# Starfish-develop/Starfish

Measured on AMD Instinct MI355X. Metric: log-likelihood evals/sec, 4096-pixel order, batch=128 walkers, higher is better.
Workload: dtype f64; 1 GPU; cfg2: synthetic single order N_pix=4096, 8 eigenspectra, M=27, N_f=8192, 1 global + 1 local kernel, all 13 parameters thawed, batch=128 walkers per GPU; global_batch=128, units_per_gpu=128, parallelism=(order x walker) units sharded x1, one process per GPU, no data-path collective

## Files before the change

include/starfish_amd.h:

```cpp
#ifndef STARFISH_AMD_H
#define STARFISH_AMD_H

#include <stddef.h>
#include <stdint.h>

#ifdef __cplusplus
extern "C" {
#endif

#define SF_OK 0
#define SF_EINVAL (-1)
#define SF_ENOMEM (-2)
#define SF_EHIP (-3)
#define SF_ENODEV (-4)

#define SF_INFO_OUT_OF_GRID (-1)
#define SF_INFO_BAD_VSINI (-2)
#define SF_INFO_BAD_WEIGHT_COV (-3)
#define SF_INFO_BANDWIDTH (-4)
#define SF_INFO_INTERNAL (-5)

#define SF_INFO_NAN (-6)

#define SF_JITTER 1e-10
// ... 144 lines not shown
int sf_banded_max_halfwidth(const sf_ctx* ctx);
int sf_banded_window_halfwidth(const sf_ctx* ctx);
size_t sf_banded_workspace_bytes(const sf_ctx* ctx, const sf_model_desc* model, int B, int halfwidth);
int sf_loglike_banded_batch(sf_ctx* ctx, const sf_model_desc* model, int B, const double* d_params,
                            int halfwidth, double* d_lnl, double* d_logdet, double* d_sqmah,
                            double* d_resid, double* d_log_scale, int* d_info, void* d_work,
                            size_t work_bytes, void* stream);

int sf_band_logdet_gram_batch(const double* d_band, int n, int halfwidth, int ldb, int64_t stride,
                              int batch, const double* d_rhs, int nrhs, int ldr, int64_t rhs_stride,
                              double* d_logdet, double* d_gram, int* d_info, void* stream);

int sf_profile_enable(int on);
int sf_profile_read(double* ms_by_stage, double* gemm_flops, long* gemm_launches, long* calls);

int sf_emulator_v11_build(const double* d_grid, int M, int P, int m, const double* d_hyper, const double* d_iphiphi,
                          double* d_A, int npad, int lda, void* stream);

int sf_emulator_v11_build_batch(const double* d_grid, int M, int P, int m, const double* d_hyper, int hyper_stride, int B,
                                const double* d_iphiphi, double* d_A, int npad, int lda, int64_t stride, int lower_only,
                                const double* d_w_hat, double* d_R, int ldr, void* stream);

size_t sf_emulator_loglike_workspace_bytes(int M, int m, int B);
int sf_emulator_loglike_batch(const double* d_grid, int M, int P, int m, const double* d_hyper, int hyper_stride, int B,
                              const double* d_iphiphi, const double* d_w_hat, double* d_lnl, double* d_logdet,
                              double* d_sqmah, int* d_info, void* d_work, size_t work_bytes, void* stream);

int sf_persistent_potrf(int enable);

int sf_persistent_potrf_status(long long* h_out8);

int sf_debug_cholesky_sequence(int mode);

int sf_debug_clock_probe(long long* d_out2, long long wall_ticks_100mhz, void* stream);

int sf_debug_stream_write(double* d_dst, size_t count, double value, void* stream);

#ifdef __cplusplus
}
#endif
#endif
```

starfish_amd/_lib.py:

```python

import ctypes as C
import os

_HERE = os.path.dirname(os.path.abspath(__file__))
LIB_PATH = os.path.join(_HERE, "libstarfish_amd.so")
if os.environ.get("SF_LIB_PATH"):
    import warnings

    LIB_PATH = os.environ["SF_LIB_PATH"]
    warnings.warn(f"starfish_amd: SF_LIB_PATH overrides the packaged library: loading {LIB_PATH}", RuntimeWarning)

c_double_p = C.POINTER(C.c_double)
c_int_p = C.POINTER(C.c_int)


class OrderDesc(C.Structure):
    _fields_ = [
        ("n", C.c_int32),
        ("nf", C.c_int32),
        ("m", C.c_int32),
        ("n_grid", C.c_int32),
        ("M", C.c_int32),
        ("reserved", C.c_int32),
        ("wave", c_double_p),
# ... 118 lines not shown
    ),
    "sf_emulator_joint_batch": (
        C.c_int,
        [_VP, C.POINTER(ModelDesc), C.c_int, _VP, _VP, _VP, _VP, _VP, C.c_size_t, _VP],
    ),
    "sf_loglike_batch": (
        C.c_int,
        [_VP, C.POINTER(ModelDesc), C.c_int, _VP, _VP, _VP, _VP, _VP, _VP, _VP, _VP, C.c_size_t, _VP],
    ),
    "sf_multi_workspace_bytes": (C.c_size_t, [C.POINTER(Segment), C.c_int, C.POINTER(ModelDesc)]),
    "sf_loglike_multi_batch": (
        C.c_int,
        [C.POINTER(Segment), C.c_int, C.POINTER(ModelDesc), _VP, _VP, _VP, _VP, _VP, _VP, C.c_size_t, _VP],
    ),
    "sf_multi_workspace_bytes_md": (C.c_size_t, [C.POINTER(Segment), C.c_int, C.POINTER(C.POINTER(ModelDesc))]),
    "sf_loglike_multi_batch_md": (
        C.c_int,
        [C.POINTER(Segment), C.c_int, C.POINTER(C.POINTER(ModelDesc)), _VP, _VP, _VP, _VP, _VP, _VP, C.c_size_t, _VP],
    ),
    "sf_banded_max_halfwidth": (C.c_int, [_VP]),
    "sf_banded_window_halfwidth": (C.c_int, [_VP]),
    "sf_banded_workspace_bytes": (C.c_size_t, [_VP, C.POINTER(ModelDesc), C.c_int, C.c_int]),
    "sf_loglike_banded_batch": (
        C.c_int,
        [_VP, C.POINTER(ModelDesc), C.c_int, _VP, C.c_int, _VP, _VP, _VP, _VP, _VP, _VP, _VP, C.c_size_t, _VP],
    ),
    "sf_band_logdet_gram_batch": (
        C.c_int,
        [_VP, C.c_int, C.c_int, C.c_int, C.c_int64, C.c_int, _VP, C.c_int, C.c_int, C.c_int64, _VP, _VP, _VP, _VP],
    ),
    "sf_debug_clock_probe": (C.c_int, [_VP, C.c_longlong, _VP]),
    "sf_debug_stream_write": (C.c_int, [_VP, C.c_size_t, C.c_double, _VP]),
    "sf_debug_cholesky_sequence": (C.c_int, [C.c_int]),
    "sf_persistent_potrf": (C.c_int, [C.c_int]),
    "sf_persistent_potrf_status": (C.c_int, [C.POINTER(C.c_longlong)]),
    "sf_profile_enable": (C.c_int, [C.c_int]),
    "sf_profile_read": (C.c_int, [c_double_p, c_double_p, C.POINTER(C.c_long), C.POINTER(C.c_long)]),
}

_lib = None


class StarfishAMDError(RuntimeError):
    """The HIP library is missing, no MI355X is visible, or a C-ABI call failed."""


def load():
    global _lib
    if _lib is not None:
        return _lib
    if not os.path.exists(LIB_PATH):
        raise StarfishAMDError(
            f"{LIB_PATH} not found: build it with `python -c 'import __graft_entry__ as g; g.build()'` "
            "or `make -C starfish_amd/csrc`.  There is no CPU fallback."
        )
    import torch

    lib = C.CDLL(LIB_PATH)
    for name, (res, args) in SIGNATURES.items():
        if not hasattr(lib, name):
            if os.environ.get("SF_LIB_PATH") and os.environ.get("SF_ALLOW_OLD_LIB") == "1":
                import warnings

                warnings.warn(f"starfish_amd: {LIB_PATH} lacks {name} (SF_ALLOW_OLD_LIB=1: skipped)", RuntimeWarning)
                continue
            raise StarfishAMDError(f"{LIB_PATH} does not export {name}: stale or mismatched build of the library "
# ... 27 lines not shown
```

starfish_amd/csrc/sf_chol.hip:

```cpp
#include <atomic>
#include <cstdlib>
#include <type_traits>
#include <vector>

#include "sf_common.h"
#include <stdio.h>
#include "sf_device.h"
#include "sf_chol_tile.h"
#include "sf_chol_host.h"
#include "sf_chol_unfused.h"
#include "sf_chol_diag.h"
#include "sf_chol_sync.h"
#include "sf_chol_solve.h"
#include "sf_chol_apply.h"
#include "sf_chol_panel.h"
#include "sf_chol_wide.h"
#include "sf_chol_seq.h"
#include "sf_chol_band.h"
#include "sf_chol_dataflow.h"

static std::atomic<int> g_chol_sequence{-1};
int sf_set_cholesky_sequence(int mode) {
    if (mode < -1 || mode > 4) {
        sf_set_error("cholesky sequence: -1 automatic, 0 fused panel kernel, 1 unfused, 2 wide (panel pairs), 3 wide then narrow (test aid), 4 dataflow");
        return SF_EINVAL;
    }
    g_chol_sequence.store(mode);
    return SF_OK;
}

#define SF_UNFUSED_BELOW 16
static bool sf_potrf_dataflow_auto(int n, int batch) {
    const int nt = (n + GT - 1) / GT;
    return sf_potrf_dataflow_fits(n, batch) && (long long)batch * nt <= 2048 && batch <= 128 && nt <= 65;
}
static int sf_potrf_pick(int n, int batch) {
    const int sel = g_chol_sequence.load();
    if (sel == 4 && !sf_potrf_dataflow_fits(n, batch)) return 0;
    if (sel >= 0) return sel;
    if (sf_potrf_dataflow_auto(n, batch)) return 4;
    if (n >= 2048 && (long long)batch * ((n + GT - 1) / GT) >= 3400) return 2;
// ... 27 lines not shown
```

starfish_amd/csrc/sf_chol_band.h:

```cpp
#pragma once
#include "sf_chol_host.h"
#include "sf_chol_panel.h"
#include "sf_chol_seq.h"

__global__ __launch_bounds__(256) void k_band_border_rows(const double* __restrict__ rhs0, int64_t srhs0, const double* __restrict__ rhs,
                                                          int64_t srhs, int ldr, int nrhs, int n, int nband, double* __restrict__ A,
                                                          int64_t sA, int lda) {
    const int b = blockIdx.z, r = blockIdx.y, col = blockIdx.x * 256 + threadIdx.x;
    if (col >= nband + 64) return;
    double v = 0.0;
    if (r < nrhs && col < n) v = r == 0 ? rhs0[(int64_t)b * srhs0 + col] : rhs[(int64_t)b * srhs + (int64_t)(r - 1) * ldr + col];
    A[(int64_t)b * sA + (int64_t)(nband + r) * lda + col] = v;
}
__global__ __launch_bounds__(256) void k_band_tiles_finish(const double* __restrict__ A, int64_t sA, int lda, int nband, int nrhs,
                                                           double* __restrict__ logdet, double* __restrict__ gram) {
    __shared__ double red[256];
    const int b = blockIdx.x, tid = threadIdx.x;
    const double* Ab = A + (int64_t)b * sA;
    double acc = 0.0;
    for (int i = tid; i < nband; i += 256) acc += log(Ab[(int64_t)i * lda + i]);
    red[tid] = acc;
    __syncthreads();
    for (int st = 128; st > 0; st >>= 1) {
        if (tid < st) red[tid] += red[tid + st];
// ... 31 lines not shown
    SF_LAUNCH_CHECK();

    const sf_potrf_scratch ws = sf_potrf_scratch_of(work, next, batch);
    auto launch_panel = [&](int k0, int pw, int row0, int nslab, bool border) -> int {
        sf_panel_args g = {};
        g.C = A;
        g.sC = sA;
        g.lda = lda;
        g.n = next;
        g.k0 = k0;
        g.pw = pw;
        g.row0 = row0;
        g.nslab = nslab + (border ? 1 : 0);
        g.slab_step = 1;
        g.Wt = ws.W;
        g.sW = ws.sW;
        g.kband = halfwidth > 0 ? halfwidth : 1;
        g.nband = nband;
        g.xrow0 = border ? nband : 0;
        if (nslab > 0) sf_park(g, ws);
        const long long nblk = (long long)g.nslab * batch;
        if (nblk <= 0) return SF_OK;
        void* tok;
        sf_prof_gemm_begin(s, 2.0 * (double)min(k0, halfwidth + GT) * GT * pw * (double)nblk, &tok);
        hipLaunchKernelGGL((k_chol_panel<false, 0>), dim3((unsigned)nblk), dim3(512), 0, s, g);
        sf_prof_gemm_end(tok);
        SF_LAUNCH_CHECK();
        return SF_OK;
    };
    SF_TRY(launch_panel(0, 0, 0, 1, false));
    for (int k = 0; k < nt; ++k) {
        const int k0 = k * GT;
        const int pw = (nband - k0 < GT) ? nband - k0 : GT;
        SF_TRY(sf_diag_step(ws, A, lda, sA, nullptr, 0, info, nband, k, ws.W, 0, s));
        const int last = (k + wt < nt - 1) ? k + wt : nt - 1;
        SF_TRY(launch_panel(k0, pw, (k + 1) * GT, last - k, true));
    }
    hipLaunchKernelGGL(k_band_tiles_finish, dim3(batch), dim3(256), 0, s, A, sA, lda, nband, nrhs, logdet, gram);
    SF_LAUNCH_CHECK();
    return SF_OK;
}
```

starfish_amd/csrc/sf_chol_dataflow.h:

```cpp
#pragma once
#include "sf_chol_host.h"
#include "sf_chol_diag.h"
#include "sf_chol_sync.h"
#include "sf_chol_panel.h"

struct sf_df_stage {
    int off;
    int St;
    int Sr;
    int thr_pt;
    int thr_rp;
    int dep;
    int fw;
};
struct sf_df_stage_packed {
    int off;
    unsigned short thr_pt, thr_rp, fw;
    unsigned char split;
    signed char dep;
};
static_assert(sizeof(sf_df_stage_packed) == 12, "sf_df_stage_packed");
template <class S>
__host__ __device__ __forceinline__ sf_df_stage sf_df_stage_of(S& x) {
    sf_df_stage r;
// ... 254 lines not shown
        }
        bl = __builtin_amdgcn_readfirstlane(bl);
        i = __builtin_amdgcn_readfirstlane(i);
        sp = __builtin_amdgcn_readfirstlane(sp);
        k = __builtin_amdgcn_readfirstlane(k);
        S = __builtin_amdgcn_readfirstlane(S);
        d = __builtin_amdgcn_readfirstlane(d);
        type = __builtin_amdgcn_readfirstlane(type);
        const int b = bchain >= 0 ? bchain : qcur + SF_DF_QUEUES * bl;
#ifdef SF_TUNING
        if ((a.miss_claims & 2) && type == T_C && b == 0 && k == 2) {
            if (tid == 0)
                while (sf_df_load(a.abort_flag) == 0) __builtin_amdgcn_s_sleep(64);
            __syncthreads();
            continue;
        }
#endif
        const int vb = bchain >= 0 ? (((a.batch - (b & (SF_DF_QUEUES - 1)) + SF_DF_QUEUES - 1) / SF_DF_QUEUES) == a.bq[0] ? 0 : 1) : v;
#ifdef SF_TUNING
        const long long dbg_t0 = wall_clock64();
        long long dbg_t1 = dbg_t0, dbg_top = 0;
#define SF_DF_MARK() dbg_t1 = wall_clock64()
#else
#define SF_DF_MARK()
#endif

        const auto& g = a.p;
        sf_panel_task q = {};
        q.nslab = 1;
        q.slab_step = 1;
        q.abort_flag = a.abort_flag;
        q.lds_int = s_ints + 1;
        q.sW = a.sT;
        auto Wof = [&](int kk) { return a.T + (size_t)(1 + kk) * GT * SF_LDT; };
        auto fpart = [&](int kk, int dd, int SS) {
            return a.part + 2 * region + (((int64_t)((kk & 1) * F + dd - 1) * a.batch + b) * a.pt_cap - (int64_t)b * SS) * (GT * GT);
        };
        int* fcnt = a.fp_cnt + 2 * SF_DF_FRONT_MAX * b;
        bool ok = true;
        int mode = 3, bid = b;
        if (type == T_C || type == T_FR) {
            const int kp = type == T_C ? k - 1 : k;
            const int slab = kp + d;
            if (type == T_C) {
                __builtin_amdgcn_s_setprio(2);
                q.Sout = a.T;
            }
            if (kp < 0) {
                if (tid == 0) __builtin_amdgcn_fence(__ATOMIC_ACQUIRE, "agent");
                __syncthreads();
            } else {
                const sf_df_stage stp = sf_df_stage_of(a.st[vb][kp > 0 ? kp - 1 : 0]);
                const int St = kp >= 1 ? stp.St : 0;
                q.k0 = kp * GT;
                q.pw = min(GT, n - q.k0);
                q.row0 = slab * GT;
                q.Wt = Wof(kp);
                q.ksplit = St;
                q.ktail = St > 0 ? (kp - 1) * (GT / GK) : 0;
                q.part = fpart(kp, d, St);
                bool dready = false;
                ok = sf_df_wait(kp >= 1 ? a.row_L + (size_t)b * nt + slab : nullptr, kp, a.done_top + b, kp,
                                St > 0 ? fcnt + SF_DF_FRONT_MAX * (kp & 1) + d - 1 : nullptr, stp.thr_pt - a.thr_base[vb][kp & 1][d - 1], a.done_D + b, kp + 1, &dready, a.abort_flag,
                                tid, s_ints + 1);
                if (!dready) {
                    q.wflag = a.done_D + b;
                    q.wval = kp + 1;
// ... 498 lines not shown
```

starfish_amd/csrc/sf_chol_host.h:

```cpp
#pragma once
#include "sf_chol_tile.h"

#define SF_TSKEW 40
#define SF_CHIP_WGS 512
#define SF_SPLIT_MAX 8
static size_t sf_split_region_tiles(void) { return 2 * SF_CHIP_WGS; }
__device__ __forceinline__ size_t sf_split_region_tiles_dev(void) { return 2 * SF_CHIP_WGS; }
static int sf_split_policy(long long wgs, int nk) {
    int S = 1;
    while (2 * S <= SF_SPLIT_MAX && wgs * 2 * S <= 384 && nk / (2 * S) >= 8) S *= 2;
    return S;
}
struct sf_potrf_scratch {
    double* T;
    int64_t sT;
    double* W;
    int64_t sW;
    double* part;
    int batch;
    size_t doubles;
    double* Wbuf(int i) const { return W + (size_t)i * batch * sW; }
    size_t Wdoubles() const { return 2 * (size_t)batch * sW; }
    double* Wslot(int k) const { return Wbuf((k >> 1) & 1) + (size_t)(k & 1) * GT * SF_LDT; }
};
static sf_potrf_scratch sf_potrf_scratch_of(double* work, int n, int batch) {
    sf_potrf_scratch w = {};
    const size_t b = (size_t)batch;
    w.sT = (int64_t)(n + SF_NB) * SF_LDT + SF_TSKEW;
    w.sW = (int64_t)SF_NB * SF_LDT + SF_TSKEW;
    w.batch = batch;
    const size_t oT = b * SF_LTB_DOUBLES, oW = oT + b * w.sT, opart = oW + w.Wdoubles() + 64;
    w.doubles = opart + (size_t)(SF_EXEC_GROUPS + 1) * sf_split_region_tiles() * (GT * GT);
    if (work) {
        w.T = work + oT;
        w.W = work + oW;
        w.part = work + opart;
    }
    return w;
}
size_t sf_potrf_work_doubles(int n, int batch) { return sf_potrf_scratch_of(nullptr, n, batch).doubles; }

template <class Args>
static void sf_set_gen(Args& g, const sf_gen_args* gen, int fp) {
    if (!gen) return;
    g.genY = gen->Y - fp;
    g.sY = (int64_t)gen->mpad * gen->ldy;
    g.ldy = gen->ldy;
    g.mpad = gen->mpad;
    g.tilemap = gen->tilemap;
    g.nt128 = gen->nt128;
}
template <class Args>
static Args sf_panel_frame(double* A, int n, int lda, int64_t stride, double* rhs, int ldr, const sf_gen_args* gen, int fp) {
    Args g = {};
    g.C = A;
    g.sC = stride;
// ... 31 lines not shown
```

starfish_amd/csrc/sf_chol_seq.h:

```cpp
#pragma once
#include "sf_chol_host.h"
#include "sf_chol_diag.h"
#include "sf_chol_panel.h"
#include "sf_chol_wide.h"

static int sf_check_front_pad(int fp, int n) {
    if (fp != 0 && (fp != 64 || n % GT != 64)) {
        sf_set_error("potrf: front pad %d does not fit n = %d", fp, n);
        return SF_EINVAL;
    }
    return SF_OK;
}

template <class Args>
static void sf_park(Args& g, const sf_potrf_scratch& ws) {
    g.Sout = ws.T;
    g.sS = ws.sT;
    g.ldS = SF_LDT;
}
static double sf_slab_rows(int n, int row0, int nslab, int step) {
    double rows = 0.0;
    for (int i = 0; i < nslab; ++i) {
        const int r0 = row0 + i * step * GT;
        rows += (n - r0 < GT) ? n - r0 : GT;
    }
    return rows;
}
static int sf_check_grid(long long nblk) {
    if (nblk > 0x7fffffffLL) {
        sf_set_error("panel grid too large");
        return SF_EINVAL;
    }
    return SF_OK;
}

static int sf_panel_split(int k0, int pw, int fp, long long nblk) {
    return pw > 0 ? sf_split_policy(nblk, (k0 > fp ? k0 - fp : 0) / GK) : 1;
}
static int sf_panel_step(sf_panel_args g, const sf_potrf_scratch& ws, int k0, int pw, int row0, int nslab, int step, const double* Wt,
                         bool to_scratch, hipStream_t st, int region, int phase) {
    const int n = g.n, fp = g.fp, batch = ws.batch;
    g.k0 = k0;
    g.pw = pw;
    g.row0 = row0;
    g.nslab = nslab;
    g.slab_step = step;
    g.Wt = Wt;
    g.sW = ws.sW;
    if (to_scratch) {
        sf_park(g, ws);
        g.prio = 1;
    }
    const long long nblk = (long long)nslab * batch;
    SF_TRY(sf_check_grid(nblk));
    const double rows = sf_slab_rows(n, row0, nslab, step);
    const double flops_main = 2.0 * (k0 > fp ? k0 - fp : 0) * rows * pw * batch;
    const double flops_epi = (rows * pw * (double)pw + (double)GT * rows * pw) * batch;
    const int nk = (k0 > fp ? k0 - fp : 0) / GK;
    const int S = sf_panel_split(k0, pw, fp, nblk);
    void* tok;
    if (S > 1) {
        g.ksplit = S;
        g.kchunk = (nk + S - 1) / S;
        g.part = ws.part + (size_t)region * sf_split_region_tiles() * (GT * GT);
        if (phase != 2) {
            sf_prof_gemm_begin(st, flops_main, &tok);
            hipLaunchKernelGGL((k_chol_panel<false, 1>), dim3((unsigned)(nblk * S)), dim3(512), 0, st, g);
            sf_prof_gemm_end(tok);
        }
        if (phase != 1) {
            sf_prof_gemm_begin(st, flops_epi, &tok);
            if (g.rhs)
                hipLaunchKernelGGL((k_chol_panel<true, 2>), dim3((unsigned)nblk), dim3(512), 0, st, g);
            else
                hipLaunchKernelGGL((k_chol_panel<false, 2>), dim3((unsigned)nblk), dim3(512), 0, st, g);
            sf_prof_gemm_end(tok);
        }
    } else {
        sf_prof_gemm_begin(st, flops_main + flops_epi, &tok);
        if (g.rhs)
            hipLaunchKernelGGL((k_chol_panel<true, 0>), dim3((unsigned)nblk), dim3(512), 0, st, g);
// ... 14 lines not shown
#ifdef SF_TUNING
static int sf_wide_stamps_begin(sf_wide_stamps& w) {
    if (SF_TUNE_FLAG("SF_WIDE_STAMPS")) {
        SF_HIP(hipHostMalloc((void**)&w.t, sizeof(long long) * 16 * 64));
        for (int i = 0; i < 16 * 64; ++i) w.t[i] = 0;
    }
    return SF_OK;
}
static void sf_wide_stamps_report(sf_wide_stamps& w, hipStream_t s) {
    if (!w.t) return;
    (void)hipStreamSynchronize(s);
    fprintf(stderr, "wide launches, workgroup grid/2: k nslab | prologue | K loop | solve 1 | 2b | solve 2 | store + rhs | S load + step 4 | S store + drain | total (us)\n");
    for (int i = 0; i < w.n; ++i) {
        const long long* t = w.t + 16 * i;
        fprintf(stderr, "%2d %2d |", w.k[i] / 1000, w.k[i] % 1000);
        const int seg[8][2] = {{0, 1}, {1, 2}, {2, 3}, {3, 4}, {4, 5}, {5, 6}, {6, 7}, {7, 8}};
        for (auto& sg : seg) fprintf(stderr, " %7.1f |", (t[sg[1]] - t[sg[0]]) / 100.0);
        fprintf(stderr, " %7.1f\n", (t[8] - t[0]) / 100.0);
    }
    (void)hipHostFree(w.t);
}
#else
static int sf_wide_stamps_begin(sf_wide_stamps&) { return SF_OK; }
static void sf_wide_stamps_report(sf_wide_stamps&, hipStream_t) {}
#endif

static int sf_panel_step_w(sf_panelw_args g, const sf_potrf_scratch& ws, int k, int slab0, int nslab, int step, bool park, hipStream_t st,
                           sf_wide_stamps& stamps) {
    const int n = g.n, fp = g.fp, batch = ws.batch;
    g.k0 = k * GT;
    g.row0 = slab0 * GT;
    g.nslab = nslab;
    g.slab_step = step;
    g.Wt0 = ws.Wslot(k);
    g.Wt1 = ws.Wslot(k + 1);
    g.sW = ws.sW;
    if (park) sf_park(g, ws);
    const long long nblk = (long long)nslab * batch;
    SF_TRY(sf_check_grid(nblk));
#ifdef SF_TUNING
    if (stamps.t && stamps.n < 64) {
        stamps.k[stamps.n] = k * 1000 + nslab;
        g.stamps = stamps.t + 16 * stamps.n++;
    }
#endif
    const double rows = sf_slab_rows(n, g.row0, nslab, step);
    const double kk = g.k0 > fp ? g.k0 - fp : 0;
    const double flops = (2.0 * kk * rows * GT + 2.0 * (kk + GT) * rows * GT + 2.0 * (rows * GT * (double)GT + (double)GT * rows * GT)) * batch;
    void* tok;
    sf_prof_gemm_begin(st, flops, &tok);
    if (g.rhs)
        hipLaunchKernelGGL(k_chol_panel_w<true>, dim3((unsigned)nblk), dim3(1024), SF_PANELW_LDS, st, g);
    else
        hipLaunchKernelGGL(k_chol_panel_w<false>, dim3((unsigned)nblk), dim3(1024), SF_PANELW_LDS, st, g);
    sf_prof_gemm_end(tok);
    SF_LAUNCH_CHECK();
    return SF_OK;
}

static int sf_diag_step(const sf_potrf_scratch& ws, double* A, int lda, int64_t stride, double* rhs, int ldr, int* info, int n, int k,
                        double* Wt, int fp, hipStream_t st) {
    const int k0 = k * GT;
    const int pw = (n - k0 < GT) ? n - k0 : GT;
    return sf_launch_diag128(ws.T, ws.sT, pw, info, k0 - fp, rhs ? rhs + k0 : nullptr, ldr, A + (int64_t)k0 * lda + k0, lda, stride, Wt,
                             ws.sW, ws.batch, st, k == 0 ? fp : 0);
}

struct sf_narrow_events {
    hipEvent_t d, rest[2];
};
static int sf_narrow_step(const sf_panel_args& base, const sf_potrf_scratch& ws, sf_exec* ex, int* info, int k, double* Wt, hipStream_t c,
                          const hipStream_t gs[2], const hipEvent_t last[2], hipEvent_t* e_top, sf_narrow_events* ev) {
    const int n = base.n, fp = base.fp, nt = (n + GT - 1) / GT;
    const int k0 = k * GT;
    const int pw = (n - k0 < GT) ? n - k0 : GT;
    *ev = {};
    SF_TRY(sf_diag_step(ws, base.C, base.lda, base.sC, base.rhs, base.ldr, info, n, k, Wt, fp, c));
    if (k + 1 >= nt) return SF_OK;
    SF_TRY(sf_exec_event(ex, &ev->d));
    SF_HIP(hipEventRecord(ev->d, c));
    const int gk = (k + 1) & 1;
    if (e_top && sf_panel_split(k0, pw, fp, ws.batch) > 1) {
        if (*e_top) SF_HIP(hipStreamWaitEvent(gs[gk], *e_top, 0));
        SF_TRY(sf_panel_step(base, ws, k0, pw, (k + 1) * GT, 1, 1, Wt, true, gs[gk], 0, 1));
        hipEvent_t e_part;
        SF_TRY(sf_exec_event(ex, &e_part));
        SF_HIP(hipEventRecord(e_part, gs[gk]));
        SF_HIP(hipStreamWaitEvent(c, e_part, 0));
        SF_TRY(sf_panel_step(base, ws, k0, pw, (k + 1) * GT, 1, 1, Wt, true, c, 0, 2));
    } else {
        if (last[gk]) SF_HIP(hipStreamWaitEvent(c, last[gk], 0));
        SF_TRY(sf_panel_step(base, ws, k0, pw, (k + 1) * GT, 1, 1, Wt, true, c, 0, 0));
    }
    if (e_top) {
        SF_TRY(sf_exec_event(ex, e_top));
        SF_HIP(hipEventRecord(*e_top, c));
    }
    for (int g = 0; g < 2; ++g) {
        const int first = k + 2 + (((k + 2) & 1) != g);
        if (first >= nt) continue;
        const int cnt = (nt - 1 - first) / 2 + 1;
        SF_HIP(hipStreamWaitEvent(gs[g], ev->d, 0));
        SF_TRY(sf_panel_step(base, ws, k0, pw, first * GT, cnt, 2, Wt, false, gs[g], 1 + g, 0));
        SF_TRY(sf_exec_event(ex, &ev->rest[g]));
        SF_HIP(hipEventRecord(ev->rest[g], gs[g]));
    }
    return SF_OK;
}

static int sf_launch_potrf_v2(double* A, int n, int lda, int64_t stride, int* info, const sf_potrf_scratch& ws, double* rhs,
                              int ldr, hipStream_t s, const sf_gen_args* gen, sf_exec* ex, int fp) {
    const int batch = ws.batch;
    SF_HIP(hipMemsetAsync(info, 0, sizeof(int) * (size_t)batch, s));
    SF_TRY(sf_exec_prepare(ex));
    constexpr int G = 2;
    hipStream_t c = ex->side;
    const hipStream_t gs[G] = {s, ex->grp[0]};
    SF_TRY(sf_exec_fork(ex, s, {c, gs[1]}));

    const sf_panel_args base = sf_panel_frame<sf_panel_args>(A, n, lda, stride, rhs, ldr, gen, fp);
    const int nt = (n + GT - 1) / GT;
    SF_TRY(sf_panel_step(base, ws, 0, 0, 0, 1, 1, nullptr, true, c, 0, 0));
    hipEvent_t e_epi = nullptr;
    hipEvent_t e_rest[G] = {};
    hipEvent_t e_rest_prev[G] = {};
    for (int k = 0; k < nt; ++k) {
        for (int g = 0; g < G; ++g)
            if (e_rest_prev[g]) SF_HIP(hipStreamWaitEvent(c, e_rest_prev[g], 0));
        sf_narrow_events ev;
        SF_TRY(sf_narrow_step(base, ws, ex, info, k, ws.Wbuf(k & 1), c, gs, e_rest, &e_epi, &ev));
        for (int g = 0; g < G; ++g) {
            e_rest_prev[g] = e_rest[g];
            if (ev.rest[g]) e_rest[g] = ev.rest[g];
        }
    }
    SF_TRY(sf_exec_join(ex, s, c, {e_rest[1]}));
    return SF_OK;
}

static int sf_launch_potrf_v3(double* A, int n, int lda, int64_t stride, int* info, const sf_potrf_scratch& ws, double* rhs,
                              int ldr, hipStream_t s, const sf_gen_args* gen, sf_exec* ex, bool half, int fp) {
    const int batch = ws.batch;
    static sf_dev_once attr_once;
    SF_CHECK(sf_lds_limit_once(&attr_once, 160 * 1024, {(const void*)k_chol_panel_w<true>, (const void*)k_chol_panel_w<false>}));
    SF_HIP(hipMemsetAsync(info, 0, sizeof(int) * (size_t)batch, s));
    SF_TRY(sf_exec_prepare(ex));
    hipStream_t c = ex->side, xa = ex->side;
    SF_TRY(sf_exec_fork(ex, s, {c, xa, ex->grp[0]}));
    const int nt = (n + GT - 1) / GT;

    const sf_panel_args base = sf_panel_frame<sf_panel_args>(A, n, lda, stride, rhs, ldr, gen, fp);
    const sf_panelw_args wbase = sf_panel_frame<sf_panelw_args>(A, n, lda, stride, rhs, ldr, gen, fp);
    sf_wide_stamps stamps;
    SF_TRY(sf_wide_stamps_begin(stamps));
    auto diag = [&](int k) -> int { return sf_diag_step(ws, A, lda, stride, rhs, ldr, info, n, k, ws.Wslot(k), fp, c); };

    SF_TRY(sf_panel_step(base, ws, 0, 0, 0, 1, 1, nullptr, true, c, 0, 0));
    const hipStream_t bs[2] = {s, ex->grp[0]};
    hipEvent_t e_A = nullptr;
    hipEvent_t e_last[2] = {nullptr, nullptr};
    std::vector<hipEvent_t> readers[4];
    auto wait_readers = [&](int slot) -> int {
        for (hipEvent_t e : readers[slot]) SF_HIP(hipStreamWaitEvent(c, e, 0));
        readers[slot].clear();
        return SF_OK;
    };
    int k = 0;
    for (; k < nt; k += 2) {
        if (k + 2 >= nt) break;
        if (half && k >= (nt / 4) * 2 && k > 0) break;
        if (e_A) SF_HIP(hipStreamWaitEvent(c, e_A, 0));
        SF_TRY(wait_readers(k & 3));
        SF_TRY(diag(k));
        SF_TRY(sf_panel_step(base, ws, k * GT, GT, (k + 1) * GT, 1, 1, ws.Wslot(k), true, c, 0, 0));
        SF_TRY(wait_readers((k + 1) & 3));
        SF_TRY(diag(k + 1));
        hipEvent_t e_chain;
        SF_TRY(sf_exec_event(ex, &e_chain));
        SF_HIP(hipEventRecord(e_chain, c));
        const int na = (nt - (k + 2) < 2) ? nt - (k + 2) : 2;
        SF_HIP(hipStreamWaitEvent(xa, e_chain, 0));
        for (int g = 0; g < 2; ++g)
            if (e_last[g]) SF_HIP(hipStreamWaitEvent(xa, e_last[g], 0));
        SF_TRY(sf_panel_step_w(wbase, ws, k, k + 2, na, 1, true, xa, stamps));
        SF_TRY(sf_exec_event(ex, &e_A));
        SF_HIP(hipEventRecord(e_A, xa));
        readers[k & 3].push_back(e_A);
        readers[(k + 1) & 3].push_back(e_A);
        for (int g = 0; g < 2; ++g) {
            const int first = k + 4 + g;
            if (first >= nt) continue;
            const int cnt = (nt - 1 - first) / 2 + 1;
            SF_HIP(hipStreamWaitEvent(bs[g], e_chain, 0));
            SF_TRY(sf_panel_step_w(wbase, ws, k, first, cnt, 2, false, bs[g], stamps));
            SF_TRY(sf_exec_event(ex, &e_last[g]));
            SF_HIP(hipEventRecord(e_last[g], bs[g]));
            readers[k & 3].push_back(e_last[g]);
            readers[(k + 1) & 3].push_back(e_last[g]);
        }
    }
    for (; k < nt; ++k) {
        if (e_A) {
            SF_HIP(hipStreamWaitEvent(c, e_A, 0));
            for (int g = 0; g < 2; ++g) SF_HIP(hipStreamWaitEvent(bs[g], e_A, 0));
            e_A = nullptr;
        }
        SF_TRY(wait_readers(k & 3));
        sf_narrow_events ev;
        SF_TRY(sf_narrow_step(base, ws, ex, info, k, ws.Wslot(k), c, bs, e_last, nullptr, &ev));
        for (int g = 0; g < 2; ++g)
            if (ev.rest[g]) {
                e_last[g] = ev.rest[g];
                readers[k & 3].push_back(ev.rest[g]);
            }
    }
    SF_TRY(sf_exec_join(ex, s, c, {e_A, e_last[1]}));
    sf_wide_stamps_report(stamps, s);
    return SF_OK;
}
```

starfish_amd/csrc/sf_common.h:

```cpp
#pragma once
#include <hip/hip_runtime.h>
#include <stdint.h>
#include <stddef.h>
#include <stdlib.h>
#include <atomic>
#include <initializer_list>
#include <mutex>
#include "sf_base.h"

#define SF_LEAF 64
#define SF_NB 256
#define SF_MAX_LOCAL 32
#define SF_NF_MIN_VSINI 16
#define SF_NF_MAX_VSINI 65536

typedef double sf_d4 __attribute__((ext_vector_type(4)));

#define SF_HIP(call)                                                                     \
    do {                                                                                 \
        hipError_t e_ = (call);                                                          \
        if (e_ != hipSuccess) {                                                          \
            sf_set_error("%s:%d %s -> %s", __FILE__, __LINE__, #call, hipGetErrorString(e_)); \
            return SF_EHIP;                                                              \
        }                                                                                \
// ... 61 lines not shown
    hipEvent_t* pool = nullptr;
    size_t pool_size = 0, pool_cap = 0, used = 0;
};
int sf_exec_prepare(sf_exec* ex);
int sf_exec_event(sf_exec* ex, hipEvent_t* e);
void sf_exec_release(sf_exec* ex);
sf_exec* sf_exec_thread_local(void);

void sf_prof_gemm_begin(hipStream_t s, double flops, void** tok);
void sf_prof_gemm_end(void* tok);

#define SF_LTB_DOUBLES (SF_LEAF * SF_LEAF + SF_LEAF)
#define SF_LDT (SF_NB + 16)
size_t sf_potrf_work_doubles(int n, int batch);
struct sf_gen_args {
    const double* Y;
    int mpad, ldy;
    const unsigned char* tilemap;
    int nt128;
    int fp;
};
int sf_potrf_front_pad(int n, int batch);
int sf_launch_potrf(double* A, int n, int lda, int64_t stride, int batch, int* info, double* work,
                    double* rhs, int ldr, hipStream_t s, const sf_gen_args* gen = nullptr, sf_exec* ex = nullptr);
int sf_band_tiles_lda(int nband);
size_t sf_band_tiles_doubles(int nband, int batch);
int sf_band_tiles_wt(int halfwidth);
int sf_launch_potrf_band(int n, int nband, int halfwidth, int batch, const double* rhs0, int64_t srhs0, const double* rhs,
                         int nrhs, int ldr, int64_t srhs, double* logdet, double* gram, int* info, double* tiles,
                         hipStream_t s);
int sf_set_persistent_potrf(int enable);
int sf_persistent_potrf_read_status(long long* out8);
int sf_set_cholesky_sequence(int mode);
int sf_launch_logdet_z(const double* L, int n, int lda, int64_t stride, int batch, const double* z, int ldr,
                       double* logdet, double* sqmah, hipStream_t s);
int sf_launch_logdet_sqmah(const double* L, int n, int lda, int64_t stride, int batch,
                           const double* R, int ldr, double* zscratch, double* logdet, double* sqmah, hipStream_t s);
int sf_launch_chol_apply(const double* L, int n, int lda, int64_t stride, int batch, int op, const double* rhs, int nrhs,
                         int ldr, int64_t rhs_stride, double* out, int ldo, int64_t out_stride, hipStream_t s);
int sf_launch_apply_stage(const double* rhs, int ldr, int64_t rhs_stride, const double* resid, int n, int npad, int nrhs,
                          int batch, double* stage, hipStream_t s);
int sf_launch_apply_export(const double* stage, const int* info, int n, int npad, int nrhs, int batch, double* out,
                           hipStream_t s);

int sf_launch_clock_probe(long long* out, long long wall_ticks, hipStream_t s);

struct sf_fill_args {
    const double* wave;
    const double* sigma;
    const double* Y;
    const double* params;
    double* C;
    int n, npad, lda, mpad, ldy, pstride;
    int64_t stride;
    int has_global, n_local, off_global, off_local;
    int lower_only;
    int add_jitter;
    int nout;
    int monotonic;
    int loguniform;
    unsigned char* tilemap;
    int nt128;
    int fp;
    unsigned* tilelist;
    int* tilecount;
    int list_cap;
// ... 33 lines not shown
```

starfish_amd/csrc/sf_free.cpp:

```cpp
#include <vector>

#include "sf_hostmath.h"
#include "sf_prof.h"
#include "sf_work.h"

extern "C" int sf_global_cov(const double* d_wave, int n, double amplitude, double lengthscale, double* d_out,
                             void* stream) {
    if (!d_wave || !d_out || n < 0) {
        sf_set_error("sf_global_cov: bad argument");
        return SF_EINVAL;
    }
    return sf_launch_global_cov(d_wave, n, amplitude, lengthscale, d_out, (hipStream_t)stream);
}
extern "C" int sf_local_cov(const double* d_wave, int n, double amplitude, double mu, double sigma,
                            int accumulate, double* d_out, void* stream) {
    if (!d_wave || !d_out || n < 0) {
        sf_set_error("sf_local_cov: bad argument");
        return SF_EINVAL;
    }
    return sf_launch_local_cov(d_wave, n, amplitude, mu, sigma, accumulate, d_out, (hipStream_t)stream);
}

extern "C" size_t sf_fft_workspace_bytes(int rows, int nf) {
    if (rows <= 0 || nf <= 0) return 0;
// ... 208 lines not shown
        (int64_t)hyper_stride < 1 + (int64_t)m + (int64_t)m * P || ((uintptr_t)d_work & 255)) {
        sf_set_error("sf_emulator_loglike_batch: bad argument (d_lnl, d_info and a 256-byte aligned d_work are required, "
                     "hyper_stride >= 1 + m + m P, B <= 65535)");
        return SF_EINVAL;
    }
    if (work_bytes < w.bytes) {
        sf_set_error("sf_emulator_loglike_batch: workspace of %zu bytes, %zu needed", work_bytes, w.bytes);
        return SF_ENOMEM;
    }
    hipStream_t s = (hipStream_t)stream;
    double* logdet = d_logdet ? d_logdet : w.logdet;
    double* sqmah = d_sqmah ? d_sqmah : w.sqmah;
    int rc = sf_launch_v11_build_batch(d_grid, M, P, m, d_hyper, hyper_stride, B, d_iphiphi, w.A, w.npad, w.lda, w.stride, 1, d_w_hat,
                                       w.R, w.npad, s);
    if (rc) return rc;
    rc = sf_potrf_batch(w.A, w.npad, w.lda, w.stride, B, w.info_c, w.potrf, w.potrf_bytes, stream);
    if (rc) return rc;
    rc = sf_logdet_sqmah_batch(w.A, w.npad, w.lda, w.stride, B, w.R, w.npad, w.potrf, w.potrf_bytes, logdet, sqmah, stream);
    if (rc) return rc;
    ProfScope ps(s, PS_SOLVE);
    return sf_launch_finish(B, logdet, sqmah, w.info_c, nullptr, d_lnl, d_info, s);
}

extern "C" int sf_persistent_potrf(int enable) { return sf_set_persistent_potrf(enable); }
extern "C" int sf_persistent_potrf_status(long long* h_out8) {
    if (!h_out8) {
        sf_set_error("sf_persistent_potrf_status: h_out8 is required");
        return SF_EINVAL;
    }
    return sf_persistent_potrf_read_status(h_out8);
}

extern "C" int sf_debug_cholesky_sequence(int mode) { return sf_set_cholesky_sequence(mode); }

extern "C" int sf_debug_stream_write(double* d_dst, size_t count, double value, void* stream) {
    if (!d_dst) {
        sf_set_error("sf_debug_stream_write: d_dst is required");
        return SF_EINVAL;
    }
    return sf_launch_stream_write(d_dst, count, value, (hipStream_t)stream);
}

extern "C" int sf_debug_clock_probe(long long* d_out2, long long wall_ticks_100mhz, void* stream) {
    return sf_launch_clock_probe(d_out2, wall_ticks_100mhz, (hipStream_t)stream);
}
```

Before: 2760 evals/s.

## Drive wide Cholesky through a launch plan with per-panel W tiles and lookahead

Replaces the hand-written multi-stream loop in the wide potrf path with a precomputed launch plan that lists each kernel, its stream and its cross-stream event waits. Panel W buffers move from a 4-slot rotating ring to one tile per panel in scratch, which removes the reader-tracking waits that guarded slot reuse. A new lookahead depth 2 lets wide-A start after only the first slab of the previous wide-B. The default depth is 1, so the main change by default is the dependency structure and dropping the ring waits. The cost is more scratch memory per panel and a risk of a wrong dependency if the plan misses a real hazard.

```diff
diff --git a/include/starfish_amd.h b/include/starfish_amd.h
--- a/include/starfish_amd.h
+++ b/include/starfish_amd.h
@@ -200,6 +200,8 @@
 
 int sf_debug_cholesky_sequence(int mode);
 
+int sf_debug_wide_lookahead(int depth);
+
 int sf_debug_clock_probe(long long* d_out2, long long wall_ticks_100mhz, void* stream);
 
 int sf_debug_stream_write(double* d_dst, size_t count, double value, void* stream);
diff --git a/starfish_amd/_lib.py b/starfish_amd/_lib.py
--- a/starfish_amd/_lib.py
+++ b/starfish_amd/_lib.py
@@ -174,6 +174,7 @@
     "sf_debug_clock_probe": (C.c_int, [_VP, C.c_longlong, _VP]),
     "sf_debug_stream_write": (C.c_int, [_VP, C.c_size_t, C.c_double, _VP]),
     "sf_debug_cholesky_sequence": (C.c_int, [C.c_int]),
+    "sf_debug_wide_lookahead": (C.c_int, [C.c_int]),
     "sf_persistent_potrf": (C.c_int, [C.c_int]),
     "sf_persistent_potrf_status": (C.c_int, [C.POINTER(C.c_longlong)]),
     "sf_profile_enable": (C.c_int, [C.c_int]),
diff --git a/starfish_amd/csrc/sf_chol.hip b/starfish_amd/csrc/sf_chol.hip
--- a/starfish_amd/csrc/sf_chol.hip
+++ b/starfish_amd/csrc/sf_chol.hip
@@ -7,6 +7,7 @@
 #include <stdio.h>
 #include "sf_device.h"
 #include "sf_chol_tile.h"
+#include "sf_chol_plan.h"
 #include "sf_chol_host.h"
 #include "sf_chol_unfused.h"
 #include "sf_chol_diag.h"
diff --git a/starfish_amd/csrc/sf_chol_band.h b/starfish_amd/csrc/sf_chol_band.h
--- a/starfish_amd/csrc/sf_chol_band.h
+++ b/starfish_amd/csrc/sf_chol_band.h
@@ -87,7 +87,7 @@
     for (int k = 0; k < nt; ++k) {
         const int k0 = k * GT;
         const int pw = (nband - k0 < GT) ? nband - k0 : GT;
-        SF_TRY(sf_diag_step(ws, A, lda, sA, nullptr, 0, info, nband, k, ws.W, 0, s));
+        SF_TRY(sf_diag_step(ws, A, lda, sA, nullptr, 0, info, nband, k, ws.W, ws.sW, 0, s));
         const int last = (k + wt < nt - 1) ? k + wt : nt - 1;
         SF_TRY(launch_panel(k0, pw, (k + 1) * GT, last - k, true));
     }
diff --git a/starfish_amd/csrc/sf_chol_dataflow.h b/starfish_amd/csrc/sf_chol_dataflow.h
--- a/starfish_amd/csrc/sf_chol_dataflow.h
+++ b/starfish_amd/csrc/sf_chol_dataflow.h
@@ -310,7 +310,7 @@
         q.abort_flag = a.abort_flag;
         q.lds_int = s_ints + 1;
         q.sW = a.sT;
-        auto Wof = [&](int kk) { return a.T + (size_t)(1 + kk) * GT * SF_LDT; };
+        auto Wof = [&](int kk) { return a.T + (size_t)sf_plan_w_tile(kk) * GT * SF_LDT; };
         auto fpart = [&](int kk, int dd, int SS) {
             return a.part + 2 * region + (((int64_t)((kk & 1) * F + dd - 1) * a.batch + b) * a.pt_cap - (int64_t)b * SS) * (GT * GT);
         };
diff --git a/starfish_amd/csrc/sf_chol_host.h b/starfish_amd/csrc/sf_chol_host.h
--- a/starfish_amd/csrc/sf_chol_host.h
+++ b/starfish_amd/csrc/sf_chol_host.h
@@ -1,5 +1,6 @@
 #pragma once
 #include "sf_chol_tile.h"
+#include "sf_chol_plan.h"
 
 #define SF_TSKEW 40
 #define SF_CHIP_WGS 512
@@ -21,7 +22,8 @@
     size_t doubles;
     double* Wbuf(int i) const { return W + (size_t)i * batch * sW; }
     size_t Wdoubles() const { return 2 * (size_t)batch * sW; }
-    double* Wslot(int k) const { return Wbuf((k >> 1) & 1) + (size_t)(k & 1) * GT * SF_LDT; }
+    double* Wpanel(int k) const { return T + (size_t)sf_plan_w_tile(k) * GT * SF_LDT; }
+    int64_t sWpanel() const { return sT; }
 };
 static sf_potrf_scratch sf_potrf_scratch_of(double* work, int n, int batch) {
     sf_potrf_scratch w = {};
diff --git a/starfish_amd/csrc/sf_chol_plan.h b/starfish_amd/csrc/sf_chol_plan.h
--- /dev/null
+++ b/starfish_amd/csrc/sf_chol_plan.h
@@ -0,0 +1,85 @@
+#pragma once
+#include <initializer_list>
+#include <vector>
+
+enum sf_plan_kind {
+    SF_PLAN_PARK0 = 0,
+    SF_PLAN_DIAG,
+    SF_PLAN_TOP,
+    SF_PLAN_REST,
+    SF_PLAN_WIDE_A,
+    SF_PLAN_WIDE_B,
+    SF_PLAN_JOIN
+};
+enum { SF_PLAN_ST_CALLER = 0, SF_PLAN_ST_CHAIN = 1, SF_PLAN_ST_GROUP1 = 2, SF_PLAN_STREAMS = 3 };
+#define SF_PLAN_MAX_WAIT 3
+struct sf_plan_launch {
+    int kind;
+    int k;
+    int slab0, nslab, step;
+    int stream;
+    int region;
+    int nwait;
+    int wait[SF_PLAN_MAX_WAIT];
+};
+static constexpr int sf_plan_park_tile(void) { return 0; }
+static constexpr int sf_plan_w_tile(int k) { return 1 + k; }
+
+#define SF_WIDE_LOOKAHEAD_DEFAULT 1
+static inline int sf_plan_lookahead_ok(int depth) { return depth == 1 || depth == 2; }
+
+static inline bool sf_wide_plan(int nt, int fp, bool half, int depth, std::vector<sf_plan_launch>& out) {
+    out.clear();
+    if (nt < 1 || (fp != 0 && fp != 64) || !sf_plan_lookahead_ok(depth)) return false;
+    auto add = [&](int kind, int k, int slab0, int nslab, int step, int stream, int region, std::initializer_list<int> waits) -> int {
+        sf_plan_launch l = {kind, k, slab0, nslab, step, stream, region, 0, {-1, -1, -1}};
+        for (int w : waits)
+            if (w >= 0 && out[(size_t)w].stream != stream) {
+                bool seen = false;
+                for (int i = 0; i < l.nwait; ++i) seen = seen || l.wait[i] == w;
+                if (!seen) l.wait[l.nwait++] = w;
+            }
+        out.push_back(l);
+        return (int)out.size() - 1;
+    };
+    const int C = SF_PLAN_ST_CHAIN;
+    const int gs[2] = {SF_PLAN_ST_CALLER, SF_PLAN_ST_GROUP1};
+    add(SF_PLAN_PARK0, 0, 0, 1, 1, C, 0, {});
+    int last[2] = {-1, -1};
+    int need[2] = {-1, -1};
+    int k = 0;
+    for (; k < nt; k += 2) {
+        if (k + 2 >= nt) break;
+        if (half && k >= (nt / 4) * 2 && k > 0) break;
+        add(SF_PLAN_DIAG, k, k, 1, 1, C, -1, {});
+        add(SF_PLAN_TOP, k, k + 1, 1, 1, C, 0, {});
+        const int chain = add(SF_PLAN_DIAG, k + 1, k + 1, 1, 1, C, -1, {});
+        const int na = (nt - (k + 2) < 2) ? nt - (k + 2) : 2;
+        add(SF_PLAN_WIDE_A, k, k + 2, na, 1, C, -1, {need[0], need[1]});
+        for (int g = 0; g < 2; ++g) {
+            need[g] = -1;
+            const int first = k + 4 + g;
+            if (first >= nt) continue;
+            const int cnt = (nt - 1 - first) / 2 + 1;
+            if (depth == 1 || cnt == 1) {
+                need[g] = last[g] = add(SF_PLAN_WIDE_B, k, first, cnt, 2, gs[g], -1, {chain});
+            } else {
+                need[g] = add(SF_PLAN_WIDE_B, k, first, 1, 2, gs[g], -1, {chain});
+                last[g] = add(SF_PLAN_WIDE_B, k, first + 2, cnt - 1, 2, gs[g], -1, {});
+            }
+        }
+    }
+    for (; k < nt; ++k) {
+        const int d = add(SF_PLAN_DIAG, k, k, 1, 1, C, -1, {});
+        if (k + 1 >= nt) break;
+        add(SF_PLAN_TOP, k, k + 1, 1, 1, C, 0, {last[(k + 1) & 1]});
+        for (int g = 0; g < 2; ++g) {
+            const int first = k + 2 + (((k + 2) & 1) != g);
+            if (first >= nt) continue;
+            const int cnt = (nt - 1 - first) / 2 + 1;
+            last[g] = add(SF_PLAN_REST, k, first, cnt, 2, gs[g], 1 + g, {d});
+        }
+    }
+    add(SF_PLAN_JOIN, nt, 0, 0, 1, SF_PLAN_ST_CALLER, -1, {(int)out.size() - 1, last[1]});
+    return true;
+}
diff --git a/starfish_amd/csrc/sf_chol_seq.h b/starfish_amd/csrc/sf_chol_seq.h
--- a/starfish_amd/csrc/sf_chol_seq.h
+++ b/starfish_amd/csrc/sf_chol_seq.h
@@ -1,5 +1,6 @@
 #pragma once
 #include "sf_chol_host.h"
+#include "sf_chol_plan.h"
 #include "sf_chol_diag.h"
 #include "sf_chol_panel.h"
 #include "sf_chol_wide.h"
@@ -38,7 +39,7 @@
     return pw > 0 ? sf_split_policy(nblk, (k0 > fp ? k0 - fp : 0) / GK) : 1;
 }
 static int sf_panel_step(sf_panel_args g, const sf_potrf_scratch& ws, int k0, int pw, int row0, int nslab, int step, const double* Wt,
-                         bool to_scratch, hipStream_t st, int region, int phase) {
+                         int64_t sW, bool to_scratch, hipStream_t st, int region, int phase) {
     const int n = g.n, fp = g.fp, batch = ws.batch;
     g.k0 = k0;
     g.pw = pw;
@@ -46,7 +47,7 @@
     g.nslab = nslab;
     g.slab_step = step;
     g.Wt = Wt;
-    g.sW = ws.sW;
+    g.sW = sW;
     if (to_scratch) {
         sf_park(g, ws);
         g.prio = 1;
@@ -127,9 +128,9 @@
     g.row0 = slab0 * GT;
     g.nslab = nslab;
     g.slab_step = step;
-    g.Wt0 = ws.Wslot(k);
-    g.Wt1 = ws.Wslot(k + 1);
-    g.sW = ws.sW;
+    g.Wt0 = ws.Wpanel(k);
+    g.Wt1 = ws.Wpanel(k + 1);
+    g.sW = ws.sWpanel();
     if (park) sf_park(g, ws);
     const long long nblk = (long long)nslab * batch;
     SF_TRY(sf_check_grid(nblk));
@@ -154,11 +155,11 @@
 }
 
 static int sf_diag_step(const sf_potrf_scratch& ws, double* A, int lda, int64_t stride, double* rhs, int ldr, int* info, int n, int k,
-                        double* Wt, int fp, hipStream_t st) {
+                        double* Wt, int64_t sW, int fp, hipStream_t st) {
     const int k0 = k * GT;
     const int pw = (n - k0 < GT) ? n - k0 : GT;
     return sf_launch_diag128(ws.T, ws.sT, pw, info, k0 - fp, rhs ? rhs + k0 : nullptr, ldr, A + (int64_t)k0 * lda + k0, lda, stride, Wt,
-                             ws.sW, ws.batch, st, k == 0 ? fp : 0);
+                             sW, ws.batch, st, k == 0 ? fp : 0);
 }
 
 struct sf_narrow_events {
@@ -170,22 +171,22 @@
     const int k0 = k * GT;
     const int pw = (n - k0 < GT) ? n - k0 : GT;
     *ev = {};
-    SF_TRY(sf_diag_step(ws, base.C, base.lda, base.sC, base.rhs, base.ldr, info, n, k, Wt, fp, c));
+    SF_TRY(sf_diag_step(ws, base.C, base.lda, base.sC, base.rhs, base.ldr, info, n, k, Wt, ws.sW, fp, c));
     if (k + 1 >= nt) return SF_OK;
     SF_TRY(sf_exec_event(ex, &ev->d));
     SF_HIP(hipEventRecord(ev->d, c));
     const int gk = (k + 1) & 1;
     if (e_top && sf_panel_split(k0, pw, fp, ws.batch) > 1) {
         if (*e_top) SF_HIP(hipStreamWaitEvent(gs[gk], *e_top, 0));
-        SF_TRY(sf_panel_step(base, ws, k0, pw, (k + 1) * GT, 1, 1, Wt, true, gs[gk], 0, 1));
+        SF_TRY(sf_panel_step(base, ws, k0, pw, (k + 1) * GT, 1, 1, Wt, ws.sW, true, gs[gk], 0, 1));
         hipEvent_t e_part;
         SF_TRY(sf_exec_event(ex, &e_part));
         SF_HIP(hipEventRecord(e_part, gs[gk]));
         SF_HIP(hipStreamWaitEvent(c, e_part, 0));
-        SF_TRY(sf_panel_step(base, ws, k0, pw, (k + 1) * GT, 1, 1, Wt, true, c, 0, 2));
+        SF_TRY(sf_panel_step(base, ws, k0, pw, (k + 1) * GT, 1, 1, Wt, ws.sW, true, c, 0, 2));
     } else {
         if (last[gk]) SF_HIP(hipStreamWaitEvent(c, last[gk], 0));
-        SF_TRY(sf_panel_step(base, ws, k0, pw, (k + 1) * GT, 1, 1, Wt, true, c, 0, 0));
+        SF_TRY(sf_panel_step(base, ws, k0, pw, (k + 1) * GT, 1, 1, Wt, ws.sW, true, c, 0, 0));
     }
     if (e_top) {
         SF_TRY(sf_exec_event(ex, e_top));
@@ -196,7 +197,7 @@
         if (first >= nt) continue;
         const int cnt = (nt - 1 - first) / 2 + 1;
         SF_HIP(hipStreamWaitEvent(gs[g], ev->d, 0));
-        SF_TRY(sf_panel_step(base, ws, k0, pw, first * GT, cnt, 2, Wt, false, gs[g], 1 + g, 0));
+        SF_TRY(sf_panel_step(base, ws, k0, pw, first * GT, cnt, 2, Wt, ws.sW, false, gs[g], 1 + g, 0));
         SF_TRY(sf_exec_event(ex, &ev->rest[g]));
         SF_HIP(hipEventRecord(ev->rest[g], gs[g]));
     }
@@ -215,7 +216,7 @@
 
     const sf_panel_args base = sf_panel_frame<sf_panel_args>(A, n, lda, stride, rhs, ldr, gen, fp);
     const int nt = (n + GT - 1) / GT;
-    SF_TRY(sf_panel_step(base, ws, 0, 0, 0, 1, 1, nullptr, true, c, 0, 0));
+    SF_TRY(sf_panel_step(base, ws, 0, 0, 0, 1, 1, nullptr, ws.sW, true, c, 0, 0));
     hipEvent_t e_epi = nullptr;
     hipEvent_t e_rest[G] = {};
     hipEvent_t e_rest_prev[G] = {};
@@ -233,83 +234,73 @@
     return SF_OK;
 }
 
+static std::atomic<int> g_wide_lookahead{SF_WIDE_LOOKAHEAD_DEFAULT};
+int sf_set_wide_lookahead(int depth) {
+    if (depth == -1) depth = SF_WIDE_LOOKAHEAD_DEFAULT;
+    if (!sf_plan_lookahead_ok(depth)) {
+        sf_set_error("wide lookahead: -1 default (%d), 1 A(p) waits for all of B(p-1), 2 for its first slabs only", SF_WIDE_LOOKAHEAD_DEFAULT);
+        return SF_EINVAL;
+    }
+    g_wide_lookahead.store(depth);
+    return SF_OK;
+}
 static int sf_launch_potrf_v3(double* A, int n, int lda, int64_t stride, int* info, const sf_potrf_scratch& ws, double* rhs,
                               int ldr, hipStream_t s, const sf_gen_args* gen, sf_exec* ex, bool half, int fp) {
     const int batch = ws.batch;
     static sf_dev_once attr_once;
     SF_CHECK(sf_lds_limit_once(&attr_once, 160 * 1024, {(const void*)k_chol_panel_w<true>, (const void*)k_chol_panel_w<false>}));
+    const int nt = (n + GT - 1) / GT;
+    std::vector<sf_plan_launch> plan;
+    if (!sf_wide_plan(nt, fp, half, g_wide_lookahead.load(), plan)) {
+        sf_set_error("potrf: no wide launch plan for %d panels in frame %d", nt, fp);
+        return SF_EINVAL;
+    }
     SF_HIP(hipMemsetAsync(info, 0, sizeof(int) * (size_t)batch, s));
     SF_TRY(sf_exec_prepare(ex));
-    hipStream_t c = ex->side, xa = ex->side;
-    SF_TRY(sf_exec_fork(ex, s, {c, xa, ex->grp[0]}));
-    const int nt = (n + GT - 1) / GT;
+    hipStream_t st[SF_PLAN_STREAMS];
+    st[SF_PLAN_ST_CALLER] = s;
+    st[SF_PLAN_ST_CHAIN] = ex->side;
+    st[SF_PLAN_ST_GROUP1] = ex->grp[0];
+    SF_TRY(sf_exec_fork(ex, s, {st[SF_PLAN_ST_CHAIN], st[SF_PLAN_ST_GROUP1]}));
 
     const sf_panel_args base = sf_panel_frame<sf_panel_args>(A, n, lda, stride, rhs, ldr, gen, fp);
     const sf_panelw_args wbase = sf_panel_frame<sf_panelw_args>(A, n, lda, stride, rhs, ldr, gen, fp);
     sf_wide_stamps stamps;
     SF_TRY(sf_wide_stamps_begin(stamps));
-    auto diag = [&](int k) -> int { return sf_diag_step(ws, A, lda, stride, rhs, ldr, info, n, k, ws.Wslot(k), fp, c); };
-
-    SF_TRY(sf_panel_step(base, ws, 0, 0, 0, 1, 1, nullptr, true, c, 0, 0));
-    const hipStream_t bs[2] = {s, ex->grp[0]};
-    hipEvent_t e_A = nullptr;
-    hipEvent_t e_last[2] = {nullptr, nullptr};
-    std::vector<hipEvent_t> readers[4];
-    auto wait_readers = [&](int slot) -> int {
-        for (hipEvent_t e : readers[slot]) SF_HIP(hipStreamWaitEvent(c, e, 0));
-        readers[slot].clear();
-        return SF_OK;
-    };
-    int k = 0;
-    for (; k < nt; k += 2) {
-        if (k + 2 >= nt) break;
-        if (half && k >= (nt / 4) * 2 && k > 0) break;
-        if (e_A) SF_HIP(hipStreamWaitEvent(c, e_A, 0));
-        SF_TRY(wait_readers(k & 3));
-        SF_TRY(diag(k));
-        SF_TRY(sf_panel_step(base, ws, k * GT, GT, (k + 1) * GT, 1, 1, ws.Wslot(k), true, c, 0, 0));
-        SF_TRY(wait_readers((k + 1) & 3));
-        SF_TRY(diag(k + 1));
-        hipEvent_t e_chain;
-        SF_TRY(sf_exec_event(ex, &e_chain));
-        SF_HIP(hipEventRecord(e_chain, c));
-        const int na = (nt - (k + 2) < 2) ? nt - (k + 2) : 2;
-        SF_HIP(hipStreamWaitEvent(xa, e_chain, 0));
-        for (int g = 0; g < 2; ++g)
-            if (e_last[g]) SF_HIP(hipStreamWaitEvent(xa, e_last[g], 0));
-        SF_TRY(sf_panel_step_w(wbase, ws, k, k + 2, na, 1, true, xa, stamps));
-        SF_TRY(sf_exec_event(ex, &e_A));
-        SF_HIP(hipEventRecord(e_A, xa));
-        readers[k & 3].push_back(e_A);
-        readers[(k + 1) & 3].push_back(e_A);
-        for (int g = 0; g < 2; ++g) {
-            const int first = k + 4 + g;
-            if (first >= nt) continue;
-            const int cnt = (nt - 1 - first) / 2 + 1;
-            SF_HIP(hipStreamWaitEvent(bs[g], e_chain, 0));
-            SF_TRY(sf_panel_step_w(wbase, ws, k, first, cnt, 2, false, bs[g], stamps));
-            SF_TRY(sf_exec_event(ex, &e_last[g]));
-            SF_HIP(hipEventRecord(e_last[g], bs[g]));
-            readers[k & 3].push_back(e_last[g]);
-            readers[(k + 1) & 3].push_back(e_last[g]);
-        }
-    }
-    for (; k < nt; ++k) {
-        if (e_A) {
-            SF_HIP(hipStreamWaitEvent(c, e_A, 0));
-            for (int g = 0; g < 2; ++g) SF_HIP(hipStreamWaitEvent(bs[g], e_A, 0));
-            e_A = nullptr;
-        }
-        SF_TRY(wait_readers(k & 3));
-        sf_narrow_events ev;
-        SF_TRY(sf_narrow_step(base, ws, ex, info, k, ws.Wslot(k), c, bs, e_last, nullptr, &ev));
-        for (int g = 0; g < 2; ++g)
-            if (ev.rest[g]) {
-                e_last[g] = ev.rest[g];
-                readers[k & 3].push_back(ev.rest[g]);
-            }
-    }
-    SF_TRY(sf_exec_join(ex, s, c, {e_A, e_last[1]}));
+    const int64_t sW = ws.sWpanel();
+
+    std::vector<hipEvent_t> done(plan.size(), nullptr);
+    std::vector<char> awaited(plan.size(), 0);
+    for (const sf_plan_launch& l : plan)
+        for (int i = 0; i < l.nwait; ++i) awaited[(size_t)l.wait[i]] = 1;
+    for (size_t i = 0; i < plan.size(); ++i) {
+        const sf_plan_launch& l = plan[i];
+        hipStream_t q = st[l.stream];
+        for (int j = 0; j < l.nwait; ++j) SF_HIP(hipStreamWaitEvent(q, done[(size_t)l.wait[j]], 0));
+        switch (l.kind) {
+            case SF_PLAN_PARK0:
+                SF_TRY(sf_panel_step(base, ws, 0, 0, 0, 1, 1, nullptr, sW, true, q, l.region, 0));
+                break;
+            case SF_PLAN_DIAG:
+                SF_TRY(sf_diag_step(ws, A, lda, stride, rhs, ldr, info, n, l.k, ws.Wpanel(l.k), sW, fp, q));
+                break;
+            case SF_PLAN_TOP:
+            case SF_PLAN_REST:
+                SF_TRY(sf_panel_step(base, ws, l.k * GT, GT, l.slab0 * GT, l.nslab, l.step, ws.Wpanel(l.k), sW, l.kind == SF_PLAN_TOP, q,
+                                     l.region, 0));
+                break;
+            case SF_PLAN_WIDE_A:
+            case SF_PLAN_WIDE_B:
+                SF_TRY(sf_panel_step_w(wbase, ws, l.k, l.slab0, l.nslab, l.step, l.kind == SF_PLAN_WIDE_A, q, stamps));
+                break;
+            default:
+                break;
+        }
+        if (awaited[i]) {
+            SF_TRY(sf_exec_event(ex, &done[i]));
+            SF_HIP(hipEventRecord(done[i], q));
+        }
+    }
     sf_wide_stamps_report(stamps, s);
     return SF_OK;
 }
diff --git a/starfish_amd/csrc/sf_common.h b/starfish_amd/csrc/sf_common.h
--- a/starfish_amd/csrc/sf_common.h
+++ b/starfish_amd/csrc/sf_common.h
@@ -117,6 +117,7 @@
 int sf_set_persistent_potrf(int enable);
 int sf_persistent_potrf_read_status(long long* out8);
 int sf_set_cholesky_sequence(int mode);
+int sf_set_wide_lookahead(int depth);
 int sf_launch_logdet_z(const double* L, int n, int lda, int64_t stride, int batch, const double* z, int ldr,
                        double* logdet, double* sqmah, hipStream_t s);
 int sf_launch_logdet_sqmah(const double* L, int n, int lda, int64_t stride, int batch,
diff --git a/starfish_amd/csrc/sf_free.cpp b/starfish_amd/csrc/sf_free.cpp
--- a/starfish_amd/csrc/sf_free.cpp
+++ b/starfish_amd/csrc/sf_free.cpp
@@ -264,6 +264,7 @@
 }
 
 extern "C" int sf_debug_cholesky_sequence(int mode) { return sf_set_cholesky_sequence(mode); }
+extern "C" int sf_debug_wide_lookahead(int depth) { return sf_set_wide_lookahead(depth); }
 
 extern "C" int sf_debug_stream_write(double* d_dst, size_t count, double value, void* stream) {
     if (!d_dst) {
```

Result: no change. 2771 evals/s, median of 6 (+0.4%).
